# tanm-ast/video-diffusion-experiments

Hardware: AMD Instinct MI355X
Metric: denoising steps/sec (whole node) at 16-frame 512×512 bf16; 1/2/4/8-GPU scaling (higher is better)
Workload: dtype bf16; 1 GPU; BASELINE config 3: AnimateDiff UNetMotionModel (SD-1.5 + motion-adapter-v1-5-2 shapes, 1.31B params), 16 frames x 64x64 latents (512x512), CFG batch 2, guidance 7.5, DDIM 50-step schedule, one hipGraph replay per step; model=UNetMotionModel[full], frames=16, latent_hw=64, global_batch=2, seq_len=4096, parallelism=single-GPU, hipgraph=True

## Files before the change

### video-diffusion-experiments_amd/csrc/ff.hip

```cpp
#include "gemm_common.h"

namespace {

constexpr int FF_C = 320, FF_H = 1280, FF_NW = 8;
constexpr int FF_KS = FF_C / 32, FF_NB = FF_C / 16, FF_NCH = FF_H / 32;
constexpr int FF_W1_SUB = 64 * 128;
constexpr int FF_W1_BYTES = (FF_C / 64) * FF_W1_SUB;
constexpr int FF_W2_BYTES = FF_C * 64;
constexpr int FF_STAGE = FF_W1_BYTES + FF_W2_BYTES;
constexpr int FF_VEC = (4 * FF_H + FF_C) * 4;
constexpr int FF_OROW = 160 * 2 + 16;
static_assert(FF_NW * 16 * FF_OROW <= FF_STAGE, "output staging reuses one ring stage");
static_assert(2 * FF_STAGE + FF_VEC <= 160 * 1024, "LDS");

struct FfArgs {
  const bf16_t* x; const bf16_t* w1; const bf16_t* w2; const bf16_t* res; bf16_t* out;
  const float* b1; const float* b2; const float* s;
  int M, ldx, ld_res, ldc;
  float eps;
  uint32_t x_bytes, res_bytes, out_bytes;
};

__device__ __forceinline__ void dma16(__amdgpu_buffer_rsrc_t r, char* lds, uint32_t voff, uint32_t soff) {
  __builtin_amdgcn_raw_ptr_buffer_load_lds(r, (lds_void*)lds, 16, voff, soff, 0, 0);
}

template <bool LNF>
__global__ __launch_bounds__(FF_NW * 64, 1) void ff_fused_kernel(const FfArgs a) {
  __shared__ __attribute__((aligned(1024))) char smem[2 * FF_STAGE + FF_VEC];
  float* sbh = (float*)(smem + 2 * FF_STAGE);
  float* sbg = sbh + FF_H;
  float* ssh = sbg + FF_H;
  float* ssg = ssh + FF_H;
  float* sb2 = ssg + FF_H;
  const int tid = threadIdx.x, lane = tid & 63;
  const int wid = __builtin_amdgcn_readfirstlane(tid >> 6);
  const int xcd = blockIdx.x & 7, j = blockIdx.x >> 3, PX = gridDim.x >> 3;
  const int M = a.M;
  const int rbs = (M + 15) / 16;
  const int rb0 = (int)((int64_t)rbs * xcd / 8), rb1 = (int)((int64_t)rbs * (xcd + 1) / 8);
  const int first = rb0 + j * FF_NW;
  if (first >= rb1) return;
  const int passes = (rb1 - first + PX * FF_NW - 1) / (PX * FF_NW);

  const __amdgpu_buffer_rsrc_t rw1 =
      __builtin_amdgcn_make_buffer_rsrc((void*)a.w1, 0, (uint32_t)(2 * FF_H * FF_C * 2), 0x00020000);
  const __amdgpu_buffer_rsrc_t rw2 =
      __builtin_amdgcn_make_buffer_rsrc((void*)a.w2, 0, (uint32_t)(FF_C * FF_H * 2), 0x00020000);
  const __amdgpu_buffer_rsrc_t rx = __builtin_amdgcn_make_buffer_rsrc((void*)a.x, 0, a.x_bytes, 0x00020000);
  const __amdgpu_buffer_rsrc_t rr =
      __builtin_amdgcn_make_buffer_rsrc((void*)(a.res ? a.res : a.x), 0, a.res ? a.res_bytes : 0u, 0x00020000);
  const __amdgpu_buffer_rsrc_t ro = __builtin_amdgcn_make_buffer_rsrc((void*)a.out, 0, a.out_bytes, 0x00020000);

  uint32_t w1off, w2off[3];
  int w2pc[3];
  {
    const int rb = lane >> 3;
    const int l = 8 * wid + rb;
    const int b = l >> 4, p = b >> 1, hg = b & 1, r = l & 15;
    const int prow = 32 * (r >> 3) + 16 * hg + 8 * ((r >> 2) & 1) + 4 * p + (r & 3);
    w1off = (uint32_t)(prow * (FF_C * 2) + (((lane & 7) ^ rb) * 16));
    w2pc[0] = wid; w2pc[1] = 8 + wid; w2pc[2] = wid < 4 ? 16 + wid : 8 + wid;
#pragma unroll
    for (int q = 0; q < 3; ++q) w2off[q] = (uint32_t)((16 * w2pc[q] + (lane & 15)) * (FF_H * 2) + (lane >> 4) * 16);
  }
  auto issue = [&](int c, int stage) {
    char* sb = smem + stage * FF_STAGE;
    const uint32_t so1 = (uint32_t)c * (uint32_t)(64 * FF_C * 2), so2 = (uint32_t)c * 64u;
#pragma unroll
    for (int s = 0; s < FF_C / 64; ++s) dma16(rw1, sb + s * FF_W1_SUB + wid * 1024, w1off + (uint32_t)(s * 128), so1);
#pragma unroll
    for (int q = 0; q < 3; ++q) dma16(rw2, sb + FF_W1_BYTES + w2pc[q] * 1024, w2off[q], so2);
  };
  issue(0, 0);
  for (int H = tid; H < FF_H; H += FF_NW * 64) {
    const int ph = 32 * (H >> 4) + (H & 15);
    sbh[H] = a.b1 ? a.b1[ph] : 0.f;
    sbg[H] = a.b1 ? a.b1[ph + 16] : 0.f;
    ssh[H] = LNF ? a.s[ph] : 0.f;
    ssg[H] = LNF ? a.s[ph + 16] : 0.f;
  }
  if (tid < FF_C) sb2[tid] = a.b2 ? a.b2[tid] : 0.f;

  const int fr = lane & 15, fq = lane >> 4;
  const int wcol = 16 * (fq & 1) + 8 * (fq >> 1);
  const uint32_t wl = (uint32_t)(fr * 128 + ((fq ^ (fr & 7)) << 4));
  bf16x8 x[FF_KS];
  auto load_x = [&](int rb) {
    const int m = rb * 16 + fr;
    const uint32_t o = (rb < rb1 && m < M) ? (uint32_t)m * (uint32_t)(a.ldx * 2) + (uint32_t)(fq * 16) : G2_OOB;
#pragma unroll
    for (int ks = 0; ks < FF_KS; ++ks)
      x[ks] = __builtin_bit_cast(bf16x8, __builtin_amdgcn_raw_buffer_load_b128(rx, o + (uint32_t)(ks * 64), 0, 0));
  };
  int r = first + wid;
  load_x(r);
  char* obuf = smem + FF_STAGE + wid * 16 * FF_OROW;

  for (int t = 0; t < passes; ++t) {
    float nmean = 0.f, rstd = 1.f;
    if constexpr (LNF) {
      f32x4 sacc = f32x4{0.f, 0.f, 0.f, 0.f}, gacc = f32x4{0.f, 0.f, 0.f, 0.f};
      const bf16x8 ones = __builtin_bit_cast(bf16x8, make_uint4(0x3F803F80u, 0x3F803F80u, 0x3F803F80u, 0x3F803F80u));
#pragma unroll
      for (int ks = 0; ks < FF_KS; ++ks) {
        sacc = __builtin_amdgcn_mfma_f32_16x16x32_bf16(ones, x[ks], sacc, 0, 0, 0);
        gacc = __builtin_amdgcn_mfma_f32_16x16x32_bf16(x[ks], x[ks], gacc, 0, 0, 0);
      }
      const int j3 = fr & 3;
      const float gd = j3 == 0 ? gacc[0] : j3 == 1 ? gacc[1] : j3 == 2 ? gacc[2] : gacc[3];
      const float sxx = __shfl(gd, fr + 16 * (fr >> 2), 64);
      constexpr float RK = 1.0f / (float)FF_C;
      const float mean = sacc[0] * RK;
      const float var = fmaf(sxx, RK, -mean * mean);
      rstd = rsqrtf(row_var_guarded<FF_KS>(x, mean, var, RK) + a.eps);
      nmean = -mean;
    }
#pragma unroll
    for (int ks = 0; ks < FF_KS; ++ks) asm volatile("" : "+v"(x[ks]));
    f32x4 acc[FF_NB];
#pragma unroll
    for (int n = 0; n < FF_NB; ++n) acc[n] = f32x4{0.f, 0.f, 0.f, 0.f};

#pragma unroll 1
    for (int c = 0; c < FF_NCH; ++c) {
      const int stage = c & 1;
      asm volatile("s_waitcnt vmcnt(0) lgkmcnt(0)" ::: "memory");
      __builtin_amdgcn_s_barrier();
      float4 tbh[2], tbg[2], tsh[2], tsg[2];
#pragma unroll
      for (int p = 0; p < 2; ++p) {
        const int H0 = 32 * c + 8 * fq + 4 * p;
        tbh[p] = *(const float4*)(sbh + H0);
        tbg[p] = *(const float4*)(sbg + H0);
        if constexpr (LNF) {
          tsh[p] = *(const float4*)(ssh + H0);
          tsg[p] = *(const float4*)(ssg + H0);
        }
      }
      __builtin_amdgcn_sched_barrier(0);
      if (c + 1 < FF_NCH) issue(c + 1, stage ^ 1);
      else if (t + 1 < passes) issue(0, 0);
      const char* sb = smem + stage * FF_STAGE;
      f32x4 hg[4];
#pragma unroll
      for (int b = 0; b < 4; ++b) hg[b] = f32x4{0.f, 0.f, 0.f, 0.f};
      bf16x8 wf[3][4];
      auto read_w1 = [&](bf16x8 (&f)[4], int ks) {
        const char* p = sb + (ks >> 1) * FF_W1_SUB + ((ks & 1) ? (wl ^ 64u) : wl);
#pragma unroll
        for (int b = 0; b < 4; ++b) f[b] = *(const bf16x8*)(p + b * 2048);
      };
      read_w1(wf[0], 0);
      read_w1(wf[1], 1);
#pragma unroll
      for (int ks = 0; ks < FF_KS; ++ks) {
        if (ks + 2 < FF_KS) read_w1(wf[(ks + 2) % 3], ks + 2);
#pragma unroll
        for (int b = 0; b < 4; ++b) hg[b] = __builtin_amdgcn_mfma_f32_16x16x32_bf16(wf[ks % 3][b], x[ks], hg[b], 0, 0, 0);
        __builtin_amdgcn_sched_barrier(0);
      }
      const char* s2 = sb + FF_W1_BYTES + lane * 16;
      constexpr int NA = 6, NBB = FF_NB - NA;
      bf16x8 w2a[NA], w2b[NBB];
#pragma unroll
      for (int n = 0; n < NA; ++n) w2a[n] = *(const bf16x8*)(s2 + n * 1024);
      if (c == FF_NCH - 1 && t + 1 < passes) load_x(r + PX * FF_NW);
      uint32_t hb[4];
#pragma unroll
      for (int p = 0; p < 2; ++p) {
        const float4 th = tbh[p], tg = tbg[p];
        const float thv[4] = {th.x, th.y, th.z, th.w}, tgv[4] = {tg.x, tg.y, tg.z, tg.w};
        float hv[4], gv[4];
        if constexpr (LNF) {
          const float4 sh = tsh[p], sg = tsg[p];
          const float shv[4] = {sh.x, sh.y, sh.z, sh.w}, sgv[4] = {sg.x, sg.y, sg.z, sg.w};
#pragma unroll
          for (int j4 = 0; j4 < 4; ++j4) {
            hv[j4] = fmaf(rstd, fmaf(nmean, shv[j4], hg[2 * p][j4]), thv[j4]);
            gv[j4] = fmaf(rstd, fmaf(nmean, sgv[j4], hg[2 * p + 1][j4]), tgv[j4]);
          }
        } else {
#pragma unroll
          for (int j4 = 0; j4 < 4; ++j4) {
            hv[j4] = hg[2 * p][j4] + thv[j4];
            gv[j4] = hg[2 * p + 1][j4] + tgv[j4];
          }
        }
#pragma unroll
        for (int h2 = 0; h2 < 2; ++h2) {
          const f32x2 go = gelu_erf2(f32x2{gv[2 * h2], gv[2 * h2 + 1]});
          const f32x2 oo = f32x2{hv[2 * h2], hv[2 * h2 + 1]} * go;
          hb[2 * p + h2] = pack2(oo[0], oo[1]);
        }
      }
      const bf16x8 hf = __builtin_bit_cast(bf16x8, make_uint4(hb[0], hb[1], hb[2], hb[3]));
      __builtin_amdgcn_sched_barrier(0);
#pragma unroll
      for (int n = 0; n < NBB; ++n) w2b[n] = *(const bf16x8*)(s2 + (NA + n) * 1024);
#pragma unroll
      for (int n = 0; n < NA; ++n) acc[n] = __builtin_amdgcn_mfma_f32_16x16x32_bf16(w2a[n], hf, acc[n], 0, 0, 0);
#pragma unroll
      for (int n = 0; n < NBB; ++n) acc[NA + n] = __builtin_amdgcn_mfma_f32_16x16x32_bf16(w2b[n], hf, acc[NA + n], 0, 0, 0);
      __builtin_amdgcn_sched_barrier(0);
    }
    u32x4 rsv[FF_NB / 2];
    {
      const int m = r * 16 + fr;
#pragma unroll
      for (int pr = 0; pr < FF_NB / 2; ++pr) {
        const uint32_t off = (r < rb1 && m < M) ? (uint32_t)(m * a.ld_res + pr * 32 + wcol) * 2u : G2_OOB;
        rsv[pr] = __builtin_amdgcn_raw_buffer_load_b128(rr, off, 0, 0);
      }
    }
    asm volatile("s_waitcnt lgkmcnt(0)" ::: "memory");
    __builtin_amdgcn_s_barrier();
#pragma unroll
    for (int half = 0; half < 2; ++half) {
#pragma unroll
      for (int n = half * (FF_NB / 2); n < (half + 1) * (FF_NB / 2); n += 2) {
        const int cc = n * 16 + wcol;
        const float4 t0 = *(const float4*)(sb2 + cc), t1 = *(const float4*)(sb2 + cc + 4);
        const float bv[8] = {t0.x, t0.y, t0.z, t0.w, t1.x, t1.y, t1.z, t1.w};
        float o[8];
#pragma unroll
        for (int jj = 0; jj < 4; ++jj) {
          auto rp = __builtin_amdgcn_permlane16_swap(__float_as_uint(acc[n][jj]), __float_as_uint(acc[n + 1][jj]),
                                                     false, false);
          o[jj] = __uint_as_float(rp[0]) + bv[jj];
          o[4 + jj] = __uint_as_float(rp[1]) + bv[4 + jj];
        }
        if (a.res) {
          float rf[8];
          const u32x4 rv = rsv[n / 2];
          unpack8(make_uint4(rv[0], rv[1], rv[2], rv[3]), rf);
#pragma unroll
          for (int jj = 0; jj < 8; ++jj) o[jj] += rf[jj];
        }
        *(uint4*)(obuf + fr * FF_OROW + (cc - half * 160) * 2) = pack8(o);
      }
      asm volatile("s_waitcnt lgkmcnt(0)" ::: "memory");
#pragma unroll
      for (int it = 0; it < 5; ++it) {
        const int q = it * 64 + lane, row = q / 20, ch = q - row * 20;
        const uint4 v = *(const uint4*)(obuf + row * FF_OROW + ch * 16);
        const int m = r * 16 + row;
        const uint32_t off = (r < rb1 && m < M) ? (uint32_t)(m * a.ldc + half * 160 + ch * 8) * 2u : G2_OOB;
        __builtin_amdgcn_raw_buffer_store_b128(u32x4{v.x, v.y, v.z, v.w}, ro, off, 0, 0);
      }
      asm volatile("s_waitcnt lgkmcnt(0)" ::: "memory");
    }
    r += PX * FF_NW;
  }
}

inline bool al16(const void* p) { return ((uintptr_t)p & 15) == 0; }

int ff_num_cus() {
  static const int cus = [] {
    int dev = 0, n = 0;
    if (hipGetDevice(&dev) == hipSuccess &&
        hipDeviceGetAttribute(&n, hipDeviceAttributeMultiprocessorCount, dev) == hipSuccess && n > 0)
      return n;
    return 256;
  }();
  return cus;
}

}

extern "C" int vd_ff_fused_takes(int64_t M, int64_t C, int64_t hidden) {
  return C == FF_C && hidden == FF_H && M >= 65536 && M * FF_C * 2 < (int64_t)G2_OOB;
}

extern "C" int vd_ff_fused(const void* x, int64_t ldx, int64_t M, int64_t C, int64_t hidden, const void* w1,
                           const float* b1, const float* ln_fold_s, float ln_eps, const void* w2, const float* b2,
                           const void* res, int64_t ld_res, void* out, int64_t ldc, vd_stream_t stream) {
  VD_CHECK_ARG(M >= 0 && C > 0 && hidden > 0);
  if (C != FF_C || hidden != FF_H) return VD_EUNSUPPORTED;
  if (M == 0) return VD_OK;
  VD_CHECK_ARG(x && w1 && w2 && out && al16(x) && al16(w1) && al16(w2) && al16(out));
  VD_CHECK_ARG(ldx >= FF_C && ldx % 8 == 0 && ldc >= FF_C && ldc % 8 == 0);
  VD_CHECK_ARG(!res || (al16(res) && ld_res >= FF_C && ld_res % 8 == 0));
  VD_CHECK_ARG(!b1 || al16(b1));
  VD_CHECK_ARG(!b2 || al16(b2));
  VD_CHECK_ARG(!ln_fold_s || (al16(ln_fold_s) && ln_eps >= 0.f));
  VD_CHECK_ARG(M * ldx * 2 < (int64_t)G2_OOB && M * ldc * 2 < (int64_t)G2_OOB &&
               (!res || M * ld_res * 2 < (int64_t)G2_OOB));
  FfArgs a;
  a.x = (const bf16_t*)x; a.w1 = (const bf16_t*)w1; a.w2 = (const bf16_t*)w2; a.res = (const bf16_t*)res;
  a.out = (bf16_t*)out; a.b1 = b1; a.b2 = b2; a.s = ln_fold_s;
  a.M = (int)M; a.ldx = (int)ldx; a.ld_res = (int)ld_res; a.ldc = (int)ldc;
  a.eps = ln_eps;
  a.x_bytes = (uint32_t)(((M - 1) * ldx + FF_C) * 2);
  a.res_bytes = res ? (uint32_t)(((M - 1) * ld_res + FF_C) * 2) : 0u;
  a.out_bytes = (uint32_t)(((M - 1) * ldc + FF_C) * 2);
  const int cus = ff_num_cus();
  const int per_xcd = cus >= 8 ? cus / 8 : 1;
  const dim3 grid((unsigned)(8 * per_xcd)), block(FF_NW * 64);
  hipStream_t s = (hipStream_t)stream;
  if (ln_fold_s) hipLaunchKernelGGL((ff_fused_kernel<true>), grid, block, 0, s, a);
  else hipLaunchKernelGGL((ff_fused_kernel<false>), grid, block, 0, s, a);
  return vd_launch_status();
}
```

Baseline: 21.73 denoising steps/s.

## Pair warps over two row blocks and software-pipeline FF1/FF2 through LDS exchange

Restructures the fused feed-forward kernel so each pair of warps shares two 16-row blocks. Each warp computes half of the hidden columns for both row blocks and half of the output columns, so every W1/W2 fragment read from LDS feeds two MFMAs. The GELU'd hidden chunk is exchanged through a small double-buffered LDS area, and the second GEMM for chunk c-1 is interleaved with the first GEMM's epilogue of chunk c. Weight DMA issues are spread across the k-loop, and the output staging gets an XOR swizzle. In exchange it uses more LDS and registers and adds a one-chunk pipeline lag with a drain step after the loop.

```diff
diff --git a/video-diffusion-experiments_amd/csrc/ff.hip b/video-diffusion-experiments_amd/csrc/ff.hip
--- a/video-diffusion-experiments_amd/csrc/ff.hip
+++ b/video-diffusion-experiments_amd/csrc/ff.hip
@@ -1,17 +1,22 @@
+#include <type_traits>
+
 #include "gemm_common.h"
 
 namespace {
 
 constexpr int FF_C = 320, FF_H = 1280, FF_NW = 8;
 constexpr int FF_KS = FF_C / 32, FF_NB = FF_C / 16, FF_NCH = FF_H / 32;
+constexpr int FF_HB = FF_NB / 2;
 constexpr int FF_W1_SUB = 64 * 128;
 constexpr int FF_W1_BYTES = (FF_C / 64) * FF_W1_SUB;
 constexpr int FF_W2_BYTES = FF_C * 64;
 constexpr int FF_STAGE = FF_W1_BYTES + FF_W2_BYTES;
 constexpr int FF_VEC = (4 * FF_H + FF_C) * 4;
-constexpr int FF_OROW = 160 * 2 + 16;
-static_assert(FF_NW * 16 * FF_OROW <= FF_STAGE, "output staging reuses one ring stage");
-static_assert(2 * FF_STAGE + FF_VEC <= 160 * 1024, "LDS");
+constexpr int FF_XCH = FF_NW * 1024;
+constexpr int FF_OUT = FF_NW * 16 * FF_C * 2;
+static_assert(FF_NCH % 2 == 0, "the ring's slot parity carries over from one pass to the next");
+static_assert(FF_W1_BYTES + FF_OUT <= 2 * FF_STAGE, "output staging: W2 slot 0 and stage 1");
+static_assert(2 * FF_STAGE + FF_VEC + 2 * FF_XCH <= 160 * 1024, "LDS");
 
 struct FfArgs {
   const bf16_t* x; const bf16_t* w1; const bf16_t* w2; const bf16_t* res; bf16_t* out;
@@ -27,7 +32,7 @@
 
 template <bool LNF>
 __global__ __launch_bounds__(FF_NW * 64, 1) void ff_fused_kernel(const FfArgs a) {
-  __shared__ __attribute__((aligned(1024))) char smem[2 * FF_STAGE + FF_VEC];
+  __shared__ __attribute__((aligned(1024))) char smem[2 * FF_STAGE + FF_VEC + 2 * FF_XCH];
   float* sbh = (float*)(smem + 2 * FF_STAGE);
   float* sbg = sbh + FF_H;
   float* ssh = sbg + FF_H;
@@ -35,6 +40,7 @@
   float* sb2 = ssg + FF_H;
   const int tid = threadIdx.x, lane = tid & 63;
   const int wid = __builtin_amdgcn_readfirstlane(tid >> 6);
+  const int pq = wid >> 1, pp = wid & 1;
   const int xcd = blockIdx.x & 7, j = blockIdx.x >> 3, PX = gridDim.x >> 3;
   const int M = a.M;
   const int rbs = (M + 15) / 16;
@@ -52,7 +58,7 @@
       __builtin_amdgcn_make_buffer_rsrc((void*)(a.res ? a.res : a.x), 0, a.res ? a.res_bytes : 0u, 0x00020000);
   const __amdgpu_buffer_rsrc_t ro = __builtin_amdgcn_make_buffer_rsrc((void*)a.out, 0, a.out_bytes, 0x00020000);
 
-  uint32_t w1off, w2off[3];
+  uint32_t w1off, w2off;
   int w2pc[3];
   {
     const int rb = lane >> 3;
@@ -61,18 +67,18 @@
     const int prow = 32 * (r >> 3) + 16 * hg + 8 * ((r >> 2) & 1) + 4 * p + (r & 3);
     w1off = (uint32_t)(prow * (FF_C * 2) + (((lane & 7) ^ rb) * 16));
     w2pc[0] = wid; w2pc[1] = 8 + wid; w2pc[2] = wid < 4 ? 16 + wid : 8 + wid;
-#pragma unroll
-    for (int q = 0; q < 3; ++q) w2off[q] = (uint32_t)((16 * w2pc[q] + (lane & 15)) * (FF_H * 2) + (lane >> 4) * 16);
+    w2off = (uint32_t)((lane & 15) * (FF_H * 2) + (lane >> 4) * 16);
   }
-  auto issue = [&](int c, int stage) {
-    char* sb = smem + stage * FF_STAGE;
-    const uint32_t so1 = (uint32_t)c * (uint32_t)(64 * FF_C * 2), so2 = (uint32_t)c * 64u;
-#pragma unroll
-    for (int s = 0; s < FF_C / 64; ++s) dma16(rw1, sb + s * FF_W1_SUB + wid * 1024, w1off + (uint32_t)(s * 128), so1);
-#pragma unroll
-    for (int q = 0; q < 3; ++q) dma16(rw2, sb + FF_W1_BYTES + w2pc[q] * 1024, w2off[q], so2);
+  auto issue_w1 = [&](int c, int s, uint32_t kill) {
+    dma16(rw1, smem + (c & 1) * FF_STAGE + s * FF_W1_SUB + wid * 1024, w1off | kill,
+          (uint32_t)c * (uint32_t)(64 * FF_C * 2) + (uint32_t)(s * 128));
   };
-  issue(0, 0);
+  auto issue_w2 = [&](int c, int q) {
+    dma16(rw2, smem + (c & 1) * FF_STAGE + FF_W1_BYTES + w2pc[q] * 1024, w2off,
+          (uint32_t)c * 64u + (uint32_t)(w2pc[q] * (16 * FF_H * 2)));
+  };
+#pragma unroll
+  for (int s = 0; s < FF_C / 64; ++s) issue_w1(0, s, 0u);
   for (int H = tid; H < FF_H; H += FF_NW * 64) {
     const int ph = 32 * (H >> 4) + (H & 15);
     sbh[H] = a.b1 ? a.b1[ph] : 0.f;
@@ -84,171 +90,233 @@
 
   const int fr = lane & 15, fq = lane >> 4;
   const int wcol = 16 * (fq & 1) + 8 * (fq >> 1);
-  const uint32_t wl = (uint32_t)(fr * 128 + ((fq ^ (fr & 7)) << 4));
-  bf16x8 x[FF_KS];
-  auto load_x = [&](int rb) {
-    const int m = rb * 16 + fr;
-    const uint32_t o = (rb < rb1 && m < M) ? (uint32_t)m * (uint32_t)(a.ldx * 2) + (uint32_t)(fq * 16) : G2_OOB;
+  const uint32_t wl = (uint32_t)(fr * 128 + ((fq ^ (fr & 7)) << 4)) + (uint32_t)(pp * 4096);
+  char* xch = smem + 2 * FF_STAGE + FF_VEC + pq * 2048 + lane * 16;
+  auto fresh_lane = [] {
+    int z = 0;
+    asm volatile("" : "+v"(z));
+    return (int)__builtin_amdgcn_mbcnt_hi(~0u, __builtin_amdgcn_mbcnt_lo(~0u, (uint32_t)z));
+  };
+  bf16x8 x[2][FF_KS];
+  auto load_x = [&](int k, int rb) {
+    const int ll = fresh_lane();
+    const int m = rb * 16 + (ll & 15);
+    const uint32_t o = (rb < rb1 && m < M) ? (uint32_t)m * (uint32_t)(a.ldx * 2) + (uint32_t)((ll >> 4) * 16) : G2_OOB;
 #pragma unroll
     for (int ks = 0; ks < FF_KS; ++ks)
-      x[ks] = __builtin_bit_cast(bf16x8, __builtin_amdgcn_raw_buffer_load_b128(rx, o + (uint32_t)(ks * 64), 0, 0));
+      x[k][ks] = __builtin_bit_cast(bf16x8, __builtin_amdgcn_raw_buffer_load_b128(rx, o + (uint32_t)(ks * 64), 0, 0));
   };
-  int r = first + wid;
-  load_x(r);
-  char* obuf = smem + FF_STAGE + wid * 16 * FF_OROW;
+  int r = first + 2 * pq;
+  load_x(0, r);
+  load_x(1, r + 1);
 
   for (int t = 0; t < passes; ++t) {
-    float nmean = 0.f, rstd = 1.f;
+    float nmean[2] = {0.f, 0.f}, rstd[2] = {1.f, 1.f};
     if constexpr (LNF) {
-      f32x4 sacc = f32x4{0.f, 0.f, 0.f, 0.f}, gacc = f32x4{0.f, 0.f, 0.f, 0.f};
-      const bf16x8 ones = __builtin_bit_cast(bf16x8, make_uint4(0x3F803F80u, 0x3F803F80u, 0x3F803F80u, 0x3F803F80u));
-#pragma unroll
-      for (int ks = 0; ks < FF_KS; ++ks) {
-        sacc = __builtin_amdgcn_mfma_f32_16x16x32_bf16(ones, x[ks], sacc, 0, 0, 0);
-        gacc = __builtin_amdgcn_mfma_f32_16x16x32_bf16(x[ks], x[ks], gacc, 0, 0, 0);
-      }
-      const int j3 = fr & 3;
-      const float gd = j3 == 0 ? gacc[0] : j3 == 1 ? gacc[1] : j3 == 2 ? gacc[2] : gacc[3];
-      const float sxx = __shfl(gd, fr + 16 * (fr >> 2), 64);
-      constexpr float RK = 1.0f / (float)FF_C;
-      const float mean = sacc[0] * RK;
-      const float var = fmaf(sxx, RK, -mean * mean);
-      rstd = rsqrtf(row_var_guarded<FF_KS>(x, mean, var, RK) + a.eps);
-      nmean = -mean;
-    }
-#pragma unroll
-    for (int ks = 0; ks < FF_KS; ++ks) asm volatile("" : "+v"(x[ks]));
-    f32x4 acc[FF_NB];
-#pragma unroll
-    for (int n = 0; n < FF_NB; ++n) acc[n] = f32x4{0.f, 0.f, 0.f, 0.f};
-
-#pragma unroll 1
-    for (int c = 0; c < FF_NCH; ++c) {
-      const int stage = c & 1;
+      uint32_t one2 = 0x3F803F80u;
+      asm volatile("" : "+v"(one2));
+      const bf16x8 ones = __builtin_bit_cast(bf16x8, make_uint4(one2, one2, one2, one2));
+#pragma unroll
+      for (int k = 0; k < 2; ++k) {
+        f32x4 sacc = f32x4{0.f, 0.f, 0.f, 0.f}, gacc = f32x4{0.f, 0.f, 0.f, 0.f};
+#pragma unroll
+        for (int ks = 0; ks < FF_KS; ++ks) {
+          sacc = __builtin_amdgcn_mfma_f32_16x16x32_bf16(ones, x[k][ks], sacc, 0, 0, 0);
+          gacc = __builtin_amdgcn_mfma_f32_16x16x32_bf16(x[k][ks], x[k][ks], gacc, 0, 0, 0);
+        }
+        const int sfr = fresh_lane() & 15, j3 = sfr & 3;
+        const float gd = j3 == 0 ? gacc[0] : j3 == 1 ? gacc[1] : j3 == 2 ? gacc[2] : gacc[3];
+        const float sxx = __shfl(gd, sfr + 16 * (sfr >> 2), 64);
+        constexpr float RK = 1.0f / (float)FF_C;
+        const float mean = sacc[0] * RK;
+        const float var = fmaf(sxx, RK, -mean * mean);
+        rstd[k] = rsqrtf(row_var_guarded<FF_KS>(x[k], mean, var, RK) + a.eps);
+        nmean[k] = -mean;
+      }
+    }
+#pragma unroll
+    for (int k = 0; k < 2; ++k)
+#pragma unroll
+      for (int ks = 0; ks < FF_KS; ++ks) asm volatile("" : "+v"(x[k][ks]));
+    f32x4 acc[2][FF_HB];
+#pragma unroll
+    for (int k = 0; k < 2; ++k)
+#pragma unroll
+      for (int n = 0; n < FF_HB; ++n) acc[k][n] = f32x4{0.f, 0.f, 0.f, 0.f};
+
+    auto read_hf = [&](bf16x8 (&hf)[2], int c1) {
+#pragma unroll
+      for (int k = 0; k < 2; ++k) hf[k] = *(const bf16x8*)(xch + (c1 & 1) * FF_XCH + k * 1024);
+    };
+    auto read_w2 = [&](bf16x8 (&w2f)[FF_HB], int c1, int n0, int n1) {
+      const char* s2 = smem + (c1 & 1) * FF_STAGE + FF_W1_BYTES + pp * (FF_HB * 1024) + lane * 16;
+#pragma unroll
+      for (int n = n0; n < n1; ++n) w2f[n] = *(const bf16x8*)(s2 + n * 1024);
+    };
+    auto ff2 = [&](const bf16x8 (&w2f)[FF_HB], const bf16x8 (&hf)[2]) {
+#pragma unroll
+      for (int n = 0; n < FF_HB; ++n)
+#pragma unroll
+        for (int k = 0; k < 2; ++k) acc[k][n] = __builtin_amdgcn_mfma_f32_16x16x32_bf16(w2f[n], hf[k], acc[k][n], 0, 0, 0);
+    };
+
+    auto chunk = [&](auto is_first, int c) {
+      constexpr bool FIRST = decltype(is_first)::value;
       asm volatile("s_waitcnt vmcnt(0) lgkmcnt(0)" ::: "memory");
       __builtin_amdgcn_s_barrier();
-      float4 tbh[2], tbg[2], tsh[2], tsg[2];
-#pragma unroll
-      for (int p = 0; p < 2; ++p) {
-        const int H0 = 32 * c + 8 * fq + 4 * p;
-        tbh[p] = *(const float4*)(sbh + H0);
-        tbg[p] = *(const float4*)(sbg + H0);
-        if constexpr (LNF) {
-          tsh[p] = *(const float4*)(ssh + H0);
-          tsg[p] = *(const float4*)(ssg + H0);
-        }
-      }
+      const int H0 = 32 * c + 8 * fq + 4 * pp;
+      const float4 tbh = *(const float4*)(sbh + H0), tbg = *(const float4*)(sbg + H0);
+      float4 tsh, tsg;
+      if constexpr (LNF) {
+        tsh = *(const float4*)(ssh + H0);
+        tsg = *(const float4*)(ssg + H0);
+      }
+      bf16x8 hf[2];
+      if constexpr (!FIRST) read_hf(hf, c - 1);
       __builtin_amdgcn_sched_barrier(0);
-      if (c + 1 < FF_NCH) issue(c + 1, stage ^ 1);
-      else if (t + 1 < passes) issue(0, 0);
-      const char* sb = smem + stage * FF_STAGE;
-      f32x4 hg[4];
-#pragma unroll
-      for (int b = 0; b < 4; ++b) hg[b] = f32x4{0.f, 0.f, 0.f, 0.f};
-      bf16x8 wf[3][4];
-      auto read_w1 = [&](bf16x8 (&f)[4], int ks) {
+      const int cn = c + 1 < FF_NCH ? c + 1 : 0;
+      const uint32_t kill = (c + 1 < FF_NCH || t + 1 < passes) ? 0u : G2_OOB;
+      const char* sb = smem + (c & 1) * FF_STAGE;
+      f32x4 hg[2][2];
+#pragma unroll
+      for (int k = 0; k < 2; ++k) hg[k][0] = hg[k][1] = f32x4{0.f, 0.f, 0.f, 0.f};
+      bf16x8 wf[3][2], w2f[FF_HB];
+      auto read_w1 = [&](bf16x8 (&f)[2], int ks) {
         const char* p = sb + (ks >> 1) * FF_W1_SUB + ((ks & 1) ? (wl ^ 64u) : wl);
-#pragma unroll
-        for (int b = 0; b < 4; ++b) f[b] = *(const bf16x8*)(p + b * 2048);
+        f[0] = *(const bf16x8*)p;
+        f[1] = *(const bf16x8*)(p + 2048);
       };
       read_w1(wf[0], 0);
       read_w1(wf[1], 1);
 #pragma unroll
       for (int ks = 0; ks < FF_KS; ++ks) {
         if (ks + 2 < FF_KS) read_w1(wf[(ks + 2) % 3], ks + 2);
-#pragma unroll
-        for (int b = 0; b < 4; ++b) hg[b] = __builtin_amdgcn_mfma_f32_16x16x32_bf16(wf[ks % 3][b], x[ks], hg[b], 0, 0, 0);
+        if (ks < FF_C / 64) issue_w1(cn, (ks + j) % (FF_C / 64), kill);
+        else if (ks < FF_C / 64 + 3) issue_w2(c, ks - FF_C / 64);
+        if constexpr (!FIRST)
+          if (ks == FF_KS - 1) read_w2(w2f, c - 1, 0, FF_HB / 2);
+#pragma unroll
+        for (int b = 0; b < 2; ++b)
+#pragma unroll
+          for (int k = 0; k < 2; ++k)
+            hg[k][b] = __builtin_amdgcn_mfma_f32_16x16x32_bf16(wf[ks % 3][b], x[k][ks], hg[k][b], 0, 0, 0);
         __builtin_amdgcn_sched_barrier(0);
       }
-      const char* s2 = sb + FF_W1_BYTES + lane * 16;
-      constexpr int NA = 6, NBB = FF_NB - NA;
-      bf16x8 w2a[NA], w2b[NBB];
-#pragma unroll
-      for (int n = 0; n < NA; ++n) w2a[n] = *(const bf16x8*)(s2 + n * 1024);
-      if (c == FF_NCH - 1 && t + 1 < passes) load_x(r + PX * FF_NW);
-      uint32_t hb[4];
-#pragma unroll
-      for (int p = 0; p < 2; ++p) {
-        const float4 th = tbh[p], tg = tbg[p];
-        const float thv[4] = {th.x, th.y, th.z, th.w}, tgv[4] = {tg.x, tg.y, tg.z, tg.w};
-        float hv[4], gv[4];
-        if constexpr (LNF) {
-          const float4 sh = tsh[p], sg = tsg[p];
-          const float shv[4] = {sh.x, sh.y, sh.z, sh.w}, sgv[4] = {sg.x, sg.y, sg.z, sg.w};
-#pragma unroll
-          for (int j4 = 0; j4 < 4; ++j4) {
-            hv[j4] = fmaf(rstd, fmaf(nmean, shv[j4], hg[2 * p][j4]), thv[j4]);
-            gv[j4] = fmaf(rstd, fmaf(nmean, sgv[j4], hg[2 * p + 1][j4]), tgv[j4]);
+      if (c == FF_NCH - 1 && t + 1 < passes) {
+        load_x(0, r + PX * FF_NW);
+        load_x(1, r + PX * FF_NW + 1);
+      }
+      const float thv[4] = {tbh.x, tbh.y, tbh.z, tbh.w}, tgv[4] = {tbg.x, tbg.y, tbg.z, tbg.w};
+      uint32_t hb[2][2];
+#pragma unroll
+      for (int u = 0; u < 4; ++u) {
+        const int k = u >> 1, h2 = u & 1;
+        if constexpr (!FIRST) {
+#pragma unroll
+          for (int i = 5 * u; i < 5 * u + 5; ++i)
+            acc[i & 1][i >> 1] = __builtin_amdgcn_mfma_f32_16x16x32_bf16(w2f[i >> 1], hf[i & 1], acc[i & 1][i >> 1], 0, 0, 0);
+        }
+        float hv[2], gv[2];
+#pragma unroll
+        for (int e = 0; e < 2; ++e) {
+          const int j4 = 2 * h2 + e;
+          if constexpr (LNF) {
+            const float shv[4] = {tsh.x, tsh.y, tsh.z, tsh.w}, sgv[4] = {tsg.x, tsg.y, tsg.z, tsg.w};
+            hv[e] = fmaf(rstd[k], fmaf(nmean[k], shv[j4], hg[k][0][j4]), thv[j4]);
+            gv[e] = fmaf(rstd[k], fmaf(nmean[k], sgv[j4], hg[k][1][j4]), tgv[j4]);
+          } else {
+            hv[e] = hg[k][0][j4] + thv[j4];
+            gv[e] = hg[k][1][j4] + tgv[j4];
           }
-        } else {
-#pragma unroll
-          for (int j4 = 0; j4 < 4; ++j4) {
-            hv[j4] = hg[2 * p][j4] + thv[j4];
-            gv[j4] = hg[2 * p + 1][j4] + tgv[j4];
+        }
+        float go0 = gelu_erf(gv[0]), go1 = gelu_erf(gv[1]);
+        asm volatile("" : "+v"(go0));
+        asm volatile("" : "+v"(go1));
+        hb[k][h2] = pack2(hv[0] * go0, hv[1] * go1);
+        if constexpr (!FIRST) {
+          asm volatile("" : "+v"(hf[0]), "+v"(hf[1]), "+v"(hb[k][h2]));
+#pragma unroll
+          for (int i = 0; i < 5; ++i) {
+            __builtin_amdgcn_sched_group_barrier(0x008, 1, 0);
+            __builtin_amdgcn_sched_group_barrier(0x002, 5, 0);
           }
         }
-#pragma unroll
-        for (int h2 = 0; h2 < 2; ++h2) {
-          const f32x2 go = gelu_erf2(f32x2{gv[2 * h2], gv[2 * h2 + 1]});
-          const f32x2 oo = f32x2{hv[2 * h2], hv[2 * h2 + 1]} * go;
-          hb[2 * p + h2] = pack2(oo[0], oo[1]);
-        }
-      }
-      const bf16x8 hf = __builtin_bit_cast(bf16x8, make_uint4(hb[0], hb[1], hb[2], hb[3]));
+        __builtin_amdgcn_sched_barrier(0);
+        if constexpr (!FIRST) {
+          if (u == 0) read_w2(w2f, c - 1, FF_HB / 2, FF_HB / 2 + 2);
+          if (u == 1) read_w2(w2f, c - 1, FF_HB / 2 + 2, FF_HB);
+        }
+      }
+#pragma unroll
+      for (int k = 0; k < 2; ++k) *(uint2*)(xch + (c & 1) * FF_XCH + k * 1024 + pp * 8) = make_uint2(hb[k][0], hb[k][1]);
       __builtin_amdgcn_sched_barrier(0);
-#pragma unroll
-      for (int n = 0; n < NBB; ++n) w2b[n] = *(const bf16x8*)(s2 + (NA + n) * 1024);
-#pragma unroll
-      for (int n = 0; n < NA; ++n) acc[n] = __builtin_amdgcn_mfma_f32_16x16x32_bf16(w2a[n], hf, acc[n], 0, 0, 0);
-#pragma unroll
-      for (int n = 0; n < NBB; ++n) acc[NA + n] = __builtin_amdgcn_mfma_f32_16x16x32_bf16(w2b[n], hf, acc[NA + n], 0, 0, 0);
-      __builtin_amdgcn_sched_barrier(0);
-    }
-    u32x4 rsv[FF_NB / 2];
+    };
+    chunk(std::true_type{}, 0);
+#pragma unroll 1
+    for (int c = 1; c < FF_NCH; ++c) chunk(std::false_type{}, c);
+
+    asm volatile("s_waitcnt vmcnt(0) lgkmcnt(0)" ::: "memory");
+    __builtin_amdgcn_s_barrier();
     {
-      const int m = r * 16 + fr;
-#pragma unroll
-      for (int pr = 0; pr < FF_NB / 2; ++pr) {
-        const uint32_t off = (r < rb1 && m < M) ? (uint32_t)(m * a.ld_res + pr * 32 + wcol) * 2u : G2_OOB;
-        rsv[pr] = __builtin_amdgcn_raw_buffer_load_b128(rr, off, 0, 0);
-      }
-    }
+      bf16x8 hf[2], w2f[FF_HB];
+      read_hf(hf, FF_NCH - 1);
+      read_w2(w2f, FF_NCH - 1, 0, FF_HB);
+      ff2(w2f, hf);
+    }
+    __builtin_amdgcn_sched_barrier(0);
+    const int le = fresh_lane();
+    const int efr = le & 15, ewcol = 16 * ((le >> 4) & 1) + 8 * (le >> 5);
+    u32x4 rsv[2][FF_HB / 2];
+#pragma unroll
+    for (int k = 0; k < 2; ++k) {
+      const int m = (r + k) * 16 + efr;
+#pragma unroll
+      for (int pr = 0; pr < FF_HB / 2; ++pr) {
+        const int cc = (FF_HB * pp + 2 * pr) * 16 + ewcol;
+        const uint32_t off = (r + k < rb1 && m < M) ? (uint32_t)(m * a.ld_res + cc) * 2u : G2_OOB;
+        rsv[k][pr] = __builtin_amdgcn_raw_buffer_load_b128(rr, off, 0, 0);
+      }
+    }
+    char* obuf = smem + FF_W1_BYTES + pq * (32 * FF_C * 2);
     asm volatile("s_waitcnt lgkmcnt(0)" ::: "memory");
     __builtin_amdgcn_s_barrier();
 #pragma unroll
-    for (int half = 0; half < 2; ++half) {
-#pragma unroll
-      for (int n = half * (FF_NB / 2); n < (half + 1) * (FF_NB / 2); n += 2) {
-        const int cc = n * 16 + wcol;
+    for (int k = 0; k < 2; ++k) {
+#pragma unroll
+      for (int n = 0; n < FF_HB; n += 2) {
+        const int cc = (FF_HB * pp + n) * 16 + ewcol;
         const float4 t0 = *(const float4*)(sb2 + cc), t1 = *(const float4*)(sb2 + cc + 4);
         const float bv[8] = {t0.x, t0.y, t0.z, t0.w, t1.x, t1.y, t1.z, t1.w};
         float o[8];
 #pragma unroll
         for (int jj = 0; jj < 4; ++jj) {
-          auto rp = __builtin_amdgcn_permlane16_swap(__float_as_uint(acc[n][jj]), __float_as_uint(acc[n + 1][jj]),
+          auto rp = __builtin_amdgcn_permlane16_swap(__float_as_uint(acc[k][n][jj]), __float_as_uint(acc[k][n + 1][jj]),
                                                      false, false);
           o[jj] = __uint_as_float(rp[0]) + bv[jj];
           o[4 + jj] = __uint_as_float(rp[1]) + bv[4 + jj];
         }
         if (a.res) {
           float rf[8];
-          const u32x4 rv = rsv[n / 2];
+          const u32x4 rv = rsv[k][n / 2];
           unpack8(make_uint4(rv[0], rv[1], rv[2], rv[3]), rf);
 #pragma unroll
           for (int jj = 0; jj < 8; ++jj) o[jj] += rf[jj];
         }
-        *(uint4*)(obuf + fr * FF_OROW + (cc - half * 160) * 2) = pack8(o);
-      }
-      asm volatile("s_waitcnt lgkmcnt(0)" ::: "memory");
+        *(uint4*)(obuf + (k * 16 + efr) * (FF_C * 2) + (((cc >> 3) ^ (efr & 7)) << 4)) = pack8(o);
+      }
+    }
+    asm volatile("s_waitcnt lgkmcnt(0)" ::: "memory");
+    __builtin_amdgcn_s_barrier();
+#pragma unroll
+    for (int k = 0; k < 2; ++k) {
 #pragma unroll
       for (int it = 0; it < 5; ++it) {
-        const int q = it * 64 + lane, row = q / 20, ch = q - row * 20;
-        const uint4 v = *(const uint4*)(obuf + row * FF_OROW + ch * 16);
-        const int m = r * 16 + row;
-        const uint32_t off = (r < rb1 && m < M) ? (uint32_t)(m * a.ldc + half * 160 + ch * 8) * 2u : G2_OOB;
+        const int q = it * 64 + le, row = 8 * pp + q / 40, ch = q % 40;
+        const uint4 v = *(const uint4*)(obuf + (k * 16 + row) * (FF_C * 2) + ((ch ^ (row & 7)) << 4));
+        const int m = (r + k) * 16 + row;
+        const uint32_t off = (r + k < rb1 && m < M) ? (uint32_t)(m * a.ldc + ch * 8) * 2u : G2_OOB;
         __builtin_amdgcn_raw_buffer_store_b128(u32x4{v.x, v.y, v.z, v.w}, ro, off, 0, 0);
       }
-      asm volatile("s_waitcnt lgkmcnt(0)" ::: "memory");
     }
     r += PX * FF_NW;
   }
```

Result: no change. 21.91 denoising steps/s (median of 6 runs) (+0.8%).
